# AndreasHeger/gat

Measured on AMD Instinct MI355X. Metric: Monte Carlo samples/sec + bit-exact p-values, 10k sims, hg19-sized workspace, higher is better.
Workload: dtype u32; 1 GPU; config2: 9982 segments x 1 tracks x 9932 intervals, 24 units / 24 contigs, 10000 samples/GPU/step, nucleotide-overlap; steps_in_flight=2

## Files before the change

### gat_amd/csrc/gat_kernels.h

```cpp
#pragma once
#include "gat_device.h"
#include "gat_annotator_steps.h"

namespace gat {


struct SamplerArgs {
  const UnitDev* units;
  const int32_t* order;
  const UnitDev* units_o;
  int32_t n_units;
  int32_t batch;
  int32_t rec_stride;
  const uint2* ws;
  const uint32_t* ws_cdf;
  const uint32_t* rank_len;
  const uint32_t* ws_tree;
  const uint4* ws_rec;
  int4* st2;
  int32_t n_long;
  int32_t n_active;
  uint32_t seed;
  int64_t sample_begin;
  uint2* slab;
// ... 127 lines not shown
            nx[q] = mt[in * kWave];
          }
          if (wv < NT - 1 && k + kGroup == kRngChunk) nx[kGroup - 1] = next_old;
#pragma unroll
          for (int q = 0; q < kGroup; ++q) {
            const uint32_t y = (cur & kMtUpper) | (nx[q] & kMtLower);
            mt[(i0 + k + q) * kWave] = far[q] ^ (y >> 1) ^ ((y & 1u) ? kMtMag : 0u);
            cur = nx[q];
          }
        }
      }
      if (wv < NT - 1) {
        const int tn = NT * (s + 1) + wv + 1;
        next_old = mt[((tn % kPerBlock) * kRngChunk) * kWave];
      }
    } else {
      const int t = NT * (s - 1) + (wv - NT);
      if (t >= 0 && t < nchunks) {
        const int e0 = t * kRngChunk;
        const int cnt = rows - e0 < kRngChunk ? rows - e0 : kRngChunk;
        const uint32_t* __restrict__ src = mt + ((t % kPerBlock) * kRngChunk) * kWave;
        uint32_t* __restrict__ dst = out + (int64_t)e0 * kWave;
        for (int k = 0; k < cnt; k += kGroup) {
          uint32_t w[kGroup];
#pragma unroll
          for (int q = 0; q < kGroup; ++q) w[q] = src[(k + q) * kWave];
#pragma unroll
          for (int q = 0; q < kGroup; ++q) {
#ifndef GAT_RNG_NO_NT
            __builtin_nontemporal_store(mt_temper(w[q]), &dst[(k + q) * kWave]);
#else
            dst[(k + q) * kWave] = mt_temper(w[q]);
#endif
          }
        }
      }
    }
    __syncthreads();
  }
}

constexpr int kPlaceChunk = 8;

template <int KIND, int MODE, int SMALL, bool PIPE>
__device__ __forceinline__ void place_body(const SamplerArgs& A) {
  constexpr bool ALL_SIMPLE = MODE == 1 || MODE == 3;
  constexpr bool TREES = MODE == 2;
  constexpr bool GRID = MODE == 5;
  constexpr int kWsTab = SMALL ? 64 : kPlaceWsLds, kRankTab = MODE == 3 ? 1 : (SMALL == 1 ? 256 : kPlaceRankLds);
  constexpr int WIDE = MODE == 3 ? kPlaceWide : (MODE == 5 ? kPlaceGridTiles : 1);
  __shared__ uint4 l_ws[kWsTab];
  __shared__ uint32_t l_rank_tab[kRankTab];
  __shared__ __attribute__((aligned(8192))) uint2 l_out_all[WIDE][16][kWave];
  extern __shared__ __attribute__((aligned(16))) uint32_t l_rank_wide[];
  uint32_t* const l_rank = MODE == 3 ? l_rank_wide : l_rank_tab;
  const int lane = threadIdx.x & (kWave - 1), wv = __builtin_amdgcn_readfirstlane((int)(threadIdx.x >> 6));
  uint2 (*const l_out)[kWave] = l_out_all[wv];
  const int n_tiles = (A.batch + kWave - 1) / kWave;
  const int a = (int)(blockIdx.y + blockIdx.z * gridDim.y);
  const int sb_own = (int)blockIdx.x * WIDE + wv;
  const int sb = sb_own < n_tiles ? sb_own : n_tiles - 1;
  if (a >= A.n_active) return;
  const UnitDev* __restrict__ Up = A.units_o + a;
  const int nws = Up->n_ws;
  const uint32_t hist_total = Up->hist_total, bucket = Up->bucket, ws_total = Up->ws_total;
  const int cap = Up->slab_cap;
  const uint2* __restrict__ ws = A.ws + Up->ws_off;
  const uint32_t* __restrict__ ws_cdf = A.ws_cdf + Up->ws_off;
  const uint32_t* __restrict__ rank_len = A.rank_len + Up->rank_off;
  const int rows = A.rng_rows[a];
  const int sidx = sb * kWave + lane;
  const bool live = sb_own < n_tiles && sidx < A.batch;
  const int64_t so = GAT_REC(A, sidx, a);

  constexpr bool kind1 = KIND == 1;
  const int target = Up->n_target;
  const bool drawL = hist_total > 2;
  const bool drawP = ws_total > 1;
  if (!drawL || !drawP) {
    if (live) A.st[so] = make_int4(0, Up->ltotal, -1, 0);
    return;
  }
  const uint32_t rangeL = hist_total - 2u, maskL = 0xffffffffu >> __builtin_clz(rangeL);
  const bool drawB = bucket > 1;
  const uint32_t rangeB = bucket - 1u, maskB = drawB ? 0xffffffffu >> __builtin_clz(rangeB) : 0u;
  const uint32_t rangeP = ws_total - 1u, maskP = 0xffffffffu >> __builtin_clz(rangeP);

  {
    const int q = (4 * a) / A.n_active;
    if (q == 0) __builtin_amdgcn_s_setprio(3);
    else if (q == 1) __builtin_amdgcn_s_setprio(2);
    else if (q == 2) __builtin_amdgcn_s_setprio(1);
  }
  const bool ws_lds = nws <= kWsTab;
  const bool rank_lds = MODE == 3 || hist_total < (uint32_t)kRankTab;
  const uint32_t* __restrict__ tree_cdf = A.ws_tree + (Up->tree_cdf_off >= 0 ? Up->tree_cdf_off : 0);
  const WsTreeGeom G = ws_tree_geom(nws);
  if (!ALL_SIMPLE && ws_lds)
    for (int i = lane; i < nws; i += kWave) {
      const uint2 v = ws[i];
      l_ws[i] = make_uint4(ws_cdf[i], v.x, v.y, i > 0 ? ws[i - 1].y : 0x80000000u);
    }
  const uint2 ws0 = ws[0];
  const bool simple_shape = nws == 1 && !drawB && ws0.y - ws0.x > 1u;
  const bool simple_lds = ALL_SIMPLE || (simple_shape && rank_lds);
  if constexpr (MODE == 3) {
    for (int i = (int)threadIdx.x; i <= (int)rangeL; i += WIDE * kWave) l_rank[i] = rank_len[i + 1];
  } else if (simple_lds) {
    for (int i = lane; i <= (int)maskL && i < kRankTab; i += kWave) l_rank[i] = (uint32_t)i <= rangeL ? rank_len[i + 1] : 0u;
  } else if (rank_lds)
    for (int i = lane; i <= (int)hist_total; i += kWave) l_rank[i] = rank_len[i];
  int cshift = 0, cspan = 0;
  uint32_t cmask = 0u;
  const uint16_t* l_g16 = nullptr;
  const uint16_t* l_k16 = nullptr;
  const uint4* __restrict__ wrec = A.ws_rec + Up->ws_off;
  if constexpr (GRID) {
    if (!ws_lds) {
      const uint32_t* __restrict__ cg = A.ws_tree + Up->cgrid_off;
      cshift = (int)cg[0]; cspan = (int)cg[2];
      const int ccells = (int)cg[1], nwords = (int)cg[3];
      cmask = (1u << cshift) - 1u;
      const uint4* __restrict__ src4 = reinterpret_cast<const uint4*>(cg + kGridHeader);
      uint4* dst4 = reinterpret_cast<uint4*>(l_rank_wide);
      for (int i = (int)threadIdx.x; i < (nwords + 3) / 4; i += WIDE * kWave) dst4[i] = src4[i];
      l_g16 = reinterpret_cast<const uint16_t*>(l_rank_wide);
      l_k16 = reinterpret_cast<const uint16_t*>(l_rank_wide + (ccells + 2) / 2);
    }
  }
  __syncthreads();
  bool use_grid = false;
  int gshift = 0, gspan = 0;
  uint8_t* l_grid = reinterpret_cast<uint8_t*>(l_ws + (kWsTab - 9));
  if (!ALL_SIMPLE && ws_lds && !simple_shape && nws > 2 && nws <= kWsTab - 9) {
    const uint32_t top = ws_total - 1u;
    gshift = top >= 128u ? (32 - __builtin_clz(top)) - 7 : 0;
    const int cells = (int)(top >> gshift) + 1;
    for (int c = lane; c <= cells; c += kWave) {
      const uint32_t t = (uint32_t)c << gshift;
      int lo_ = 0, hi_ = nws;
      while (lo_ < hi_) {
        const int mid = lo_ + ((hi_ - lo_) >> 1);
        if ((int32_t)(l_ws[mid].x - t) < 0) lo_ = mid + 1; else hi_ = mid;
      }
      l_grid[c] = (uint8_t)(lo_ < nws ? lo_ : nws - 1);
    }
    __syncthreads();
    uint32_t span = 0;
    for (int c = lane; c < cells; c += kWave) span = max(span, (uint32_t)l_grid[c + 1] - (uint32_t)l_grid[c]);
    gspan = (int)wave_max_u32(span);
    use_grid = true;
  }
  const uint32_t* __restrict__ rp = A.rng_out + A.rng_off[a] + (int64_t)sb * rows * kWave + lane;
  uint2* __restrict__ out = A.slab + (int64_t)(live ? sidx : 0) * A.slab_stride + Up->slab_off;

  int32_t rem = Up->ltotal;
  int nS = 0;
  uint32_t len = 0, cs = 0, ce = 0;
  int32_t sstart = 0;
  int32_t pend = -1;
  uint32_t used = 0;
  int flag = 0;


  bool sL = live, sP = false, sO = false;
  uint32_t omaskS = 0u, orangeS = 0u;
  const int32_t c_ss = (int32_t)ws0.x + 1;
  const uint32_t c_r3 = ws0.y - ws0.x - 2u;
#define GAT_STEP_SIMPLE_B(Y, LR1, JJ)                                                                          \
  {                                                                                                            \
    const uint32_t y_ = (Y);                                                                                   \
        \
    const bool accL = (y_ & maskL) <= rangeL;                                                                  \
    const bool accP = (y_ & maskP) <= rangeP;                                                                  \
              \
    const uint32_t vO = y_ & omaskS;                                                                           \
    const bool accO = vO <= orangeS;                                                                           \
    const bool isL = sL && accL, isP = sP && accP, isO = sO && accO;                                           \
    const uint32_t range3 = c_r3 + len;                                                                        \
    omaskS = isP ? 0xffffffffu >> __builtin_clz(range3 | 1u) : omaskS;                                         \
    orangeS = isP ? range3 : orangeS;                                                                          \
    const bool trig = isL && !kind1 && rem <= (int32_t)(LR1);                         \
    const int32_t q = c_ss - (int32_t)len + (int32_t)vO;                                                       \
    const uint32_t start = (uint32_t)(q > 0 ? q : 0);                                                          \
    const uint32_t end = (uint32_t)(q + (int32_t)len);                                                         \
    const int32_t omin = (int32_t)ws0.y < (int32_t)end ? (int32_t)ws0.y : (int32_t)end;                        \
    const int32_t omax = (int32_t)ws0.x > (int32_t)start ? (int32_t)ws0.x : (int32_t)start;                    \
    const int32_t overlap = omin - omax > 0 ? omin - omax : 0;                                                 \
    const bool full = isO && nS >= cap;                                                                        \
    const bool put = isO && !full;                                                                             \
                                              \
    if (MODE == 3 || put) l_out[nS & 15][lane] = make_uint2(start, end);                                       \
    nS += put ? 1 : 0;                                                                                         \
    rem -= put ? overlap : 0;                                                                                  \
    flag |= full ? kStatusOverflow : 0;                                                                        \
    const bool fin = kind1 && put && nS == target;                                                             \
    len = isL ? (LR1) : len;                                                                                   \
    pend = trig ? (int32_t)len : (fin ? -2 : pend);                                                            \
    used = (trig || put) ? (JJ) + 1u : used;        \
    sL = (sL && !isL) || (put && !fin);                                                                        \
    sP = (sP && !isP) || (isL && !trig);                                                                       \
    sO = (sO && !isO) || isP;                                                                                  \
  }

  const uint32_t lmaxS = rank_len[1u + rangeL];
  const bool cm_ok = A.place_plain_step == 0 && (uint64_t)c_r3 + (uint64_t)lmaxS <= (uint64_t)maskP;
  uint64_t mL = 0, mP = 0, mO = 0;
  uint32_t nS9 = 0, used_lo = 0;
  const uint32_t lane_ring = (uint32_t)(size_t)(__attribute__((address_space(3))) void*)&l_out[0][lane];
#define GAT_STEP_SIMPLE_ASM(YREG, LR1, JJ1)                                                                       \
  {                                                                                                            \
    uint32_t t0_, t1_, t2_, t3_;                                                                               \
    uint64_t sa_, sb_, sc_;                                                                                    \
    asm volatile(                                                                                              \
        "v_and_b32 %7, %16, v" #YREG "\n\t"                                                     \
        "v_and_b32 %8, %26, v" #YREG "\n\t"                                                          \
        "v_cmp_ge_u32_e64 %12, %17, %7\n\t"                                            \
        "v_add_u32 %9, %19, %0\n\t"                                                            \
        "v_cmp_ge_u32 vcc, %18, %8\n\t"                                                              \
        "v_cmp_le_u32_e64 %13, %7, %9\n\t"                                         \
        "s_and_b64 %11, %4, vcc\n\t"                                                                  \
        "v_cmp_le_i32 vcc, %1, %15\n\t"                                  \
        "s_and_b64 %12, %5, %12\n\t"                                                                  \
        "s_and_b64 %13, %6, %13\n\t"                                                                  \
        "s_and_b64 vcc, %11, vcc\n\t"                         \
        "v_cndmask_b32_e64 %0, %0, %15, %11\n\t"                                 \
        "v_cndmask_b32_e64 %3, %3, %25, vcc\n\t"                    \
        "s_xor_b64 %4, %4, %11\n\t"                                                                            \
        "s_andn2_b64 %11, %11, vcc\n\t"                                                   \
        "s_xor_b64 %5, %5, %12\n\t"                                                                            \
        "s_xor_b64 %6, %6, %13\n\t"                                                                            \
        "s_or_b64 %4, %4, %13\n\t"                     \
        "s_or_b64 %5, %5, %11\n\t"                       \
        "s_or_b64 %6, %6, %12\n\t"                                     \
        "s_and_saveexec_b64 %11, %13\n\t"                                 \
        "v_add_u32 %9, %20, %7\n\t"                       \
        "v_and_or_b32 %8, %2, %23, %24\n\t"                                                     \
        "v_sub_u32 %7, %9, %0\n\t"                                                          \
        "v_add_u32 %2, 0x200, %2\n\t"                                                                          \
        "v_min_i32 %10, %22, %9\n\t"                                                     \
        "v_max_i32 %7, 0, %7\n\t"                                                       \
        "v_sub_u32 %1, %1, %10\n\t"                              \
        "v_max_i32 %10, %21, %7\n\t"                                                 \
        "ds_write2_b32 %8, %7, %9 offset1:1\n\t"                                                               \
        "v_mov_b32 %3, %25\n\t"                                                                                \
        "v_add_u32 %1, %1, %10\n\t"                                                                            \
        "s_mov_b64 exec, %11"                                                                                  \
        : "+v"(len), "+v"(rem), "+v"(nS9), "+v"(used_lo), "+s"(mL), "+s"(mP), "+s"(mO),                        \
          "=&v"(t0_), "=&v"(t1_), "=&v"(t2_), "=&v"(t3_), "=&s"(sa_), "=&s"(sb_), "=&s"(sc_)                   \
        : "n"(0), "v"(LR1), "s"(maskP), "s"(rangeP), "s"(rangeL), "s"(c_r3), "s"(c_ss), "s"(ws0.x), "s"(ws0.y), \
          "s"(0x1e00u), "v"(lane_ring), "n"(JJ1), "s"(maskL)                                                   \
        : "vcc", "scc", "memory");                                                                             \
  }

  int nF = 0;
  auto flush = [&]() __attribute__((always_inline)) {
    if (nS - nF >= 8 && nF + 8 <= cap) {
      uint4* __restrict__ dst = reinterpret_cast<uint4*>(out + nF);
      const int w0 = nF & 15;
#pragma unroll
      for (int w = 0; w < 4; ++w) {
        const uint2 e0 = l_out[w0 + 2 * w][lane], e1 = l_out[w0 + 2 * w + 1][lane];
#ifdef GAT_EXP_NO_STORES
        if (e0.x == 0xfffffff1u && e1.y == 0xfffffff2u)
#endif
        dst[w] = make_uint4(e0.x, e0.y, e1.x, e1.y);
      }
      nF += 8;
    }
  };
  bool sB = false;
  bool alive_c = true;
  uint32_t omask = 0u, orange = 0u;
#define GAT_STEP_TABLE_B(Y, LR, PCS, PCE, PPE, JJ)                                                             \
  {                                                                                                            \
    const uint32_t y_ = (Y);                                                                                   \
    const uint32_t vB = y_ & maskB, vO = y_ & omask;                                                           \
    const bool isL = sL && (y_ & maskL) <= rangeL, isB = sB && vB <= rangeB;                                   \
    const bool isP = sP && (y_ & maskP) <= rangeP, isO = sO && vO <= orange;                                   \
    len = isL ? (LR) * bucket : (isB ? len + vB : len);                                          \
    const bool have_len = drawB ? isB : isL;                                                                   \
    const bool trig = have_len && !kind1 && rem <= (int32_t)len;                      \
    cs = isP ? (PCS) : cs;                                                                                     \
    ce = isP ? (PCE) : ce;                                                                                     \
    int32_t sstartP = (int32_t)(PCS) - (int32_t)len + 1;                                         \
    sstartP = (int32_t)(PPE) > sstartP ? (int32_t)(PPE) : sstartP;                                             \
    const uint32_t range3 = (PCE) - 1u - (uint32_t)sstartP;                                                    \
    const bool placeP = isP && range3 == 0;                             \
    const bool place = isO || placeP;                                                                          \
    const int32_t q = isO ? sstart + (int32_t)vO : sstartP;                                                    \
    const uint32_t start = (uint32_t)(q > 0 ? q : 0);                                  \
    const uint32_t end = (uint32_t)(q + (int32_t)len);                                                         \
    const int32_t omin = (int32_t)ce < (int32_t)end ? (int32_t)ce : (int32_t)end;                              \
    const int32_t omax = (int32_t)cs > (int32_t)start ? (int32_t)cs : (int32_t)start;                          \
    const int32_t overlap = omin - omax > 0 ? omin - omax : 0;                                                 \
    const bool full = place && nS >= cap;                                                                      \
    const bool put = place && !full;                                                                           \
    if (put) l_out[nS & 15][lane] = make_uint2(start, end);                                                    \
    nS += put ? 1 : 0;                                                                                         \
    rem -= put ? overlap : 0;                                                                                  \
    flag |= full ? kStatusOverflow : 0;                                                                        \
    const bool fin = kind1 && put && nS == target;                                                             \
    pend = trig ? (int32_t)len : (fin ? -2 : pend);                                                            \
    used = (trig || put) ? (JJ) + 1u : used;                                                                   \
    sstart = isP ? sstartP : sstart;                                                                           \
    omask = isP ? 0xffffffffu >> __builtin_clz(range3 | 1u) : omask;                                           \
    orange = isP ? range3 : orange;                                                                            \
    sL = (sL && !isL) || (put && !fin);                                                                        \
    sB = (sB && !isB) || (isL && drawB);                                                                       \
    sP = (sP && !isP) || (have_len && !trig);                                                                  \
    sO = (sO && !isO) || (isP && !placeP);                                                                     \
  }

  uint32_t ya[kPlaceChunk], yb[kPlaceChunk], lr[kPlaceChunk] = {0, 0, 0, 0, 0, 0, 0, 0};
  uint32_t pcs[kPlaceChunk] = {0, 0, 0, 0, 0, 0, 0, 0}, pce[kPlaceChunk] = {0, 0, 0, 0, 0, 0, 0, 0},
           ppe[kPlaceChunk] = {0, 0, 0, 0, 0, 0, 0, 0};
#define GAT_STEP_TABLE_ASM(YREG, LR1, PCS, PCE, PPE, JJ1)                                                         \
  {                                                                                                            \
    uint32_t t0_, t1_, t2_, t3_;                                                                               \
    uint64_t sa_, sb_, sc_;                                                                                    \
    asm volatile(                                                                                              \
        "v_and_b32 %12, %24, v" #YREG "\n\t"                                                         \
        "v_and_b32 %13, %27, v" #YREG "\n\t"                                                         \
        "v_and_b32 %14, %8, v" #YREG "\n\t"                                    \
        "v_cmp_ge_u32_e64 %17, %25, %12\n\t"                                                         \
        "v_cmp_ge_u32 vcc, %26, %13\n\t"                                                             \
        "v_cmp_le_u32_e64 %18, %14, %9\n\t"                                         \
        "s_and_b64 %16, %4, vcc\n\t"                                                                  \
        "v_cmp_le_i32 vcc, %1, %20\n\t"                                  \
        "s_and_b64 %17, %5, %17\n\t"                                                                  \
        "s_and_b64 %18, %6, %18\n\t"                                                                  \
        "s_and_b64 vcc, %16, vcc\n\t"                                                      \
        "v_cndmask_b32_e64 %0, %0, %20, %16\n\t"                                                      \
        "v_cndmask_b32_e64 %3, %3, %30, vcc\n\t"                                                  \
        "s_xor_b64 %4, %4, %16\n\t"                                                                            \
        "s_andn2_b64 %16, %16, vcc\n\t"                                                   \
        "s_xor_b64 %5, %5, %17\n\t"                                                                            \
        "s_xor_b64 %6, %6, %18\n\t"                                                                            \
        "s_or_b64 %5, %5, %16\n\t"                               \
        "s_and_saveexec_b64 %16, %17\n\t"                       \
        "v_sub_u32 %12, %21, %0\n\t"                                                  \
        "v_mov_b32 %10, %21\n\t"                                                                       \
        "v_add_u32 %12, 1, %12\n\t"                                                                            \
        "v_mov_b32 %11, %22\n\t"                                                                       \
        "v_max_i32 %7, %23, %12\n\t"                                                       \
        "v_mov_b32 %14, 0\n\t"                              \
        "v_sub_u32 %12, %22, %7\n\t"                                                                           \
        "v_add_u32 %9, -1, %12\n\t"                    \
        "v_or_b32 %12, 1, %9\n\t"                                                                              \
        "v_ffbh_u32 %12, %12\n\t"                                                                              \
        "v_cmp_eq_u32 vcc, 0, %9\n\t"                                             \
        "v_lshrrev_b32_e64 %8, %12, -1\n\t"                                                      \
        "s_mov_b64 exec, %16\n\t"                                                                              \
        "s_andn2_b64 %17, %17, vcc\n\t"                                                 \
        "s_or_b64 %18, %18, vcc\n\t"                                                 \
        "s_or_b64 %6, %6, %17\n\t"                                           \
        "s_or_b64 %4, %4, %18\n\t"                                               \
        "s_and_saveexec_b64 %16, %18\n\t"                                                                      \
        "v_add_u32 %12, %7, %14\n\t"                                          \
        "v_and_or_b32 %13, %2, %28, %29\n\t"                                                    \
        "v_add_u32 %15, %12, %0\n\t"                                                        \
        "v_max_i32 %12, 0, %12\n\t"                                                     \
        "v_add_u32 %2, 0x200, %2\n\t"                                                                          \
        "v_min_i32 %14, %11, %15\n\t"                                                        \
        "v_sub_u32 %1, %1, %14\n\t"                                                  \
        "v_max_i32 %14, %10, %12\n\t"                                                      \
        "ds_write2_b32 %13, %12, %15 offset1:1\n\t"                                                            \
        "v_mov_b32 %3, %30\n\t"                                                                                \
        "v_add_u32 %1, %1, %14\n\t"                                                                            \
        "s_mov_b64 exec, %16"                                                                                  \
        : "+v"(len), "+v"(rem), "+v"(nS9), "+v"(used_lo), "+s"(mL), "+s"(mP), "+s"(mO),                        \
          "+v"(sstart), "+v"(omask), "+v"(orange), "+v"(cs), "+v"(ce),                                         \
          "=&v"(t0_), "=&v"(t1_), "=&v"(t2_), "=&v"(t3_), "=&s"(sa_), "=&s"(sb_), "=&s"(sc_)                   \
        : "n"(0), "v"(LR1), "v"(PCS), "v"(PCE), "v"(PPE), "s"(maskP), "s"(rangeP), "s"(rangeL), "s"(maskL),    \
          "s"(0x1e00u), "v"(lane_ring), "n"(JJ1)                                                               \
        : "vcc", "scc", "memory");                                                                             \
  }
#define GAT_PRE_RANK_L(Y)                                                                                      \
  _Pragma("unroll") for (int c = 0; c < kPlaceChunk; ++c) {                                                    \
    const uint32_t v = (Y)[c] & maskL; lr[c] = l_rank[v <= rangeL ? 1u + v : 0u]; }
#define GAT_PRE_RANK_G(Y)                                                                                      \
  _Pragma("unroll") for (int c = 0; c < kPlaceChunk; ++c) {                                                    \
    const uint32_t v = (Y)[c] & maskL; lr[c] = rank_len[v <= rangeL ? 1u + v : 0u]; }
#define GAT_PRE_WS(Y)                                                                                          \
  {                                                                                                            \
    uint32_t pv[kPlaceChunk]; int lo[kPlaceChunk];                                                             \
    _Pragma("unroll") for (int c = 0; c < kPlaceChunk; ++c) {                                                  \
      const uint32_t v = (Y)[c] & maskP; pv[c] = v <= rangeP ? v : rangeP; lo[c] = 0; }                        \
    if (use_grid) {                                                                                            \
      _Pragma("unroll") for (int c = 0; c < kPlaceChunk; ++c) lo[c] = (int)l_grid[pv[c] >> gshift];             \
    }                                                                                                          \
    for (int n = use_grid ? gspan : nws; n > 1;) {              \
      const int half = n >> 1;                                                                                 \
      _Pragma("unroll") for (int c = 0; c < kPlaceChunk; ++c) {                                                \
        const int pr = lo[c] + half - 1;                 \
        lo[c] = (int32_t)(l_ws[pr < nws ? pr : nws - 1].x - pv[c]) < 0 ? lo[c] + half : lo[c];                 \
      }                                                                                                        \
      n -= half;                                                                                               \
    }                                                                                                          \
    _Pragma("unroll") for (int c = 0; c < kPlaceChunk; ++c) {                                                  \
      uint4 w4 = l_ws[lo[c]];                                                                                  \
      if ((int32_t)(w4.x - pv[c]) < 0) w4 = l_ws[lo[c] + 1];                                                   \
      pcs[c] = w4.y; pce[c] = w4.z; ppe[c] = w4.w; }                                                           \
  }
#define GAT_PRE_WS2(Y)                                                                                         \
  {                                                                                                            \
    uint32_t pv[kPlaceChunk]; int lo[kPlaceChunk];                                                             \
    _Pragma("unroll") for (int c = 0; c < kPlaceChunk; ++c) {                                                  \
      const uint32_t v = (Y)[c] & maskP; pv[c] = v <= rangeP ? v : rangeP; }                                   \
    {                                                        \
      const uint32_t pa[4] = {pv[0], pv[1], pv[2], pv[3]}, pb[4] = {pv[4], pv[5], pv[6], pv[7]};               \
      int la[4], lb[4];                                                                                        \
      ws_tree_count<true, 4>(tree_cdf, G, pa, la);                                                             \
      ws_tree_count<true, 4>(tree_cdf, G, pb, lb);                                                             \
      _Pragma("unroll") for (int c = 0; c < 4; ++c) { lo[c] = la[c]; lo[4 + c] = lb[c]; }                      \
    }                                                                                                          \
    _Pragma("unroll") for (int c = 0; c < kPlaceChunk; ++c) {                                                  \
      const uint2 w2 = ws[lo[c]];                                                                              \
      pcs[c] = w2.x; pce[c] = w2.y; ppe[c] = lo[c] > 0 ? ws[lo[c] - 1].y : 0x80000000u; }                      \
  }
#ifdef GAT_EXP_NOGATHER
#define GAT_EXP_REC(I) ((I) & 0)
#else
// ... 212 lines not shown
    int jbase = 0;                                                                                           \
    uint32_t pcsB[kPlaceChunk], pceB[kPlaceChunk], ppeB[kPlaceChunk];                                        \
    asm volatile("; GAT_PINNED_BEGIN BASE=192" ::: "memory");                                                \
    GAT_PIN_LOAD(192, 193, 194, 195, 196, 197, 198, 199, 0)                                                  \
    GAT_PIN_LOAD(200, 201, 202, 203, 204, 205, 206, 207, kPlaceChunk)                                        \
    GAT_PIN_LOAD(208, 209, 210, 211, 212, 213, 214, 215, 2 * kPlaceChunk)                                    \
    GAT_PIN_LOAD(216, 217, 218, 219, 220, 221, 222, 223, 3 * kPlaceChunk)                                    \
    GAT_PIN_TAKE2(ya, 192, 193, 194, 195, 196, 197, 198, 199)                                                \
    alive_c = sL;                                                                                            \
    GAT_PRE_WS3X(ya, pcs, pce, ppe)                                                                          \
    for (int j = 0; j < rows; j += 4 * kPlaceChunk) {                                                        \
      if ((mL | mP | mO) == 0) break;                                                                        \
      GAT_FOLD_USED(jbase)                                                                                   \
      jbase = j;                                                                                             \
      GAT_DEEP_SUB(0, ya, pcs, pce, ppe, yb, pcsB, pceB, ppeB, 200, 201, 202, 203, 204, 205, 206, 207,        \
                   192, 193, 194, 195, 196, 197, 198, 199, j + 4 * kPlaceChunk)                               \
      if (j + 1 * kPlaceChunk >= rows || (mL | mP | mO) == 0) break;                                         \
      GAT_DEEP_SUB(1, yb, pcsB, pceB, ppeB, ya, pcs, pce, ppe, 208, 209, 210, 211, 212, 213, 214, 215,        \
                   200, 201, 202, 203, 204, 205, 206, 207, j + 5 * kPlaceChunk)                               \
      if (j + 2 * kPlaceChunk >= rows || (mL | mP | mO) == 0) break;                                         \
      GAT_DEEP_SUB(2, ya, pcs, pce, ppe, yb, pcsB, pceB, ppeB, 216, 217, 218, 219, 220, 221, 222, 223,        \
                   208, 209, 210, 211, 212, 213, 214, 215, j + 6 * kPlaceChunk)                               \
      if (j + 3 * kPlaceChunk >= rows || (mL | mP | mO) == 0) break;                                         \
      GAT_DEEP_SUB(3, yb, pcsB, pceB, ppeB, ya, pcs, pce, ppe, 192, 193, 194, 195, 196, 197, 198, 199,        \
                   216, 217, 218, 219, 220, 221, 222, 223, j + 7 * kPlaceChunk)                               \
    }                                                                                                        \
    asm volatile("s_waitcnt vmcnt(0)\n\t; GAT_PINNED_END" ::: "memory");                                     \
    GAT_FOLD_USED(jbase)                                                                                     \
    nS = (int)(nS9 >> 9);                                                                                    \
    sL = (mL >> lane) & 1; sP = (mP >> lane) & 1; sO = (mO >> lane) & 1;                                     \
  }
#define GAT_PLACE_LOOP(PRE, ONE, ALIVE)                                                                        \
  {                                                                                                            \
    const uint32_t* __restrict__ rq = rp;                                                                      \
    _Pragma("unroll") for (int c = 0; c < kPlaceChunk; ++c) ya[c] = rq[c * kWave];                             \
    for (int j = 0; j < rows; j += 2 * kPlaceChunk) {                                                          \
      if (__ballot(ALIVE) == 0) break;                                                                         \
      GAT_PSTAMP(4)                                                                                            \
      const bool more_b = j + kPlaceChunk < rows;                                                              \
      if (more_b) {                                                                                            \
        _Pragma("unroll") for (int c = 0; c < kPlaceChunk; ++c) yb[c] = rq[(kPlaceChunk + c) * kWave];         \
      }                                                                                                        \
      GAT_PSTAMP(0)                                                                                            \
      if constexpr (GRID) alive_c = (ALIVE);                                                                   \
      PRE(ya)                                                                                                  \
      GAT_PSTAMP(1)                                                                                            \
      _Pragma("unroll") for (int c = 0; c < kPlaceChunk; ++c) ONE(ya, c, (uint32_t)(j + c))                    \
      GAT_PSTAMP(2)                                                                                            \
      GAT_PSTAMP(3)                                                                                            \
      GAT_PROWS                                                                                                \
      if (!more_b || __ballot(ALIVE) == 0) break;                                                              \
      if (j + 2 * kPlaceChunk < rows) {                                                                        \
        _Pragma("unroll") for (int c = 0; c < kPlaceChunk; ++c) ya[c] = rq[(2 * kPlaceChunk + c) * kWave];     \
      }                                                                                                        \
      rq += 2 * kPlaceChunk * kWave;                                                                           \
      GAT_PSTAMP(0)                                                                                            \
      if constexpr (GRID) alive_c = (ALIVE);                                                                   \
      PRE(yb)                                                                                                  \
      GAT_PSTAMP(1)                                                                                            \
      _Pragma("unroll") for (int c = 0; c < kPlaceChunk; ++c) ONE(yb, c, (uint32_t)(j + kPlaceChunk + c))      \
      GAT_PSTAMP(2)                                                                                            \
      flush();                                                                                                 \
      GAT_PSTAMP(3)                                                                                            \
      GAT_PROWS                                                                                                \
    }                                                                                                          \
  }
  bool plain_step = true;
  if constexpr (MODE == 3) {
    static_assert(PIPE, "k_place_wide runs the hand-pipelined loop");
    if (!kind1 && cm_ok) { plain_step = false; GAT_PLACE_LOOP_PIPE_ASM(GAT_PRE_SIMPLE_W, GAT_ONE_SIMPLE_ASM) }
    else GAT_PLACE_LOOP_PIPE(GAT_PRE_SIMPLE_W, GAT_ONE_SIMPLE_B, GAT_ALIVE_B)
  } else if (simple_lds) {
    if constexpr (PIPE) {
      if (!kind1 && cm_ok) { plain_step = false; GAT_PLACE_LOOP_PIPE_ASM(GAT_PRE_SIMPLE_L, GAT_ONE_SIMPLE_ASM) }
      else GAT_PLACE_LOOP_PIPE(GAT_PRE_SIMPLE_L, GAT_ONE_SIMPLE_B, GAT_ALIVE_B)
    } else GAT_PLACE_LOOP(GAT_PRE_SIMPLE_L, GAT_ONE_SIMPLE_B, GAT_ALIVE_B)
  } else if constexpr (!ALL_SIMPLE) {
    if (simple_shape) GAT_PLACE_LOOP(GAT_PRE_SIMPLE_G, GAT_ONE_SIMPLE_B, GAT_ALIVE_B)
    else {
      if (ws_lds) {
        if (rank_lds) {
          if (!kind1 && !drawB && A.place_plain_step == 0) { plain_step = false; GAT_PLACE_LOOP_PIPE_ASM(GAT_PRE_TABLE_LL, GAT_ONE_TABLE_ASM) }
          else GAT_PLACE_LOOP(GAT_PRE_TABLE_LL, GAT_ONE_TABLE, GAT_ALIVE_TB)
        } else GAT_PLACE_LOOP(GAT_PRE_TABLE_GL, GAT_ONE_TABLE, GAT_ALIVE_TB)
      } else if constexpr (TREES) {
        if (rank_lds) GAT_PLACE_LOOP(GAT_PRE_TABLE_LG, GAT_ONE_TABLE, GAT_ALIVE_TB) else GAT_PLACE_LOOP(GAT_PRE_TABLE_GG, GAT_ONE_TABLE, GAT_ALIVE_TB)
      } else if constexpr (GRID) {
        if (rank_lds) {
          if (!kind1 && !drawB && A.place_plain_step == 0) {
            plain_step = false;
            GAT_PLACE_LOOP_DEEP_ASM
          } else GAT_PLACE_LOOP(GAT_PRE_TABLE_L3, GAT_ONE_TABLE, GAT_ALIVE_TB)
        } else GAT_PLACE_LOOP(GAT_PRE_TABLE_G3, GAT_ONE_TABLE, GAT_ALIVE_TB)
      }
    }
  }
#undef GAT_PROWS
#ifdef GAT_DIAG
  if (lane == 0 && A.diag_place != nullptr && sb_own < n_tiles) {
    for (int k = 0; k < 5; ++k) atomicAdd(&A.diag_place[(int64_t)a * 8 + k], pdg[k]);
    atomicAdd(&A.diag_place[(int64_t)a * 8 + 5], pdg_rows);
    atomicAdd(&A.diag_place[(int64_t)a * 8 + 6], 1ull);
    if (A.diag_tiles != nullptr) {
      unsigned long long tile_t1;
      asm volatile("s_memrealtime %0\n\ts_waitcnt lgkmcnt(0)" : "=s"(tile_t1) :: "memory");
      A.diag_tiles[((int64_t)a * n_tiles + sb_own) * 2] = tile_t0;
      A.diag_tiles[((int64_t)a * n_tiles + sb_own) * 2 + 1] = tile_t1;
    }
  }
#endif
#undef GAT_PLACE_LOOP
#undef GAT_PLACE_LOOP_PIPE
#undef GAT_PLACE_CHUNK
#undef GAT_PIN_TAKE
#undef GAT_PIN_LOAD
#undef GAT_ONE_TABLE
#undef GAT_ONE_SIMPLE_B
#undef GAT_ALIVE_B
#undef GAT_STEP_SIMPLE_B
#undef GAT_STEP_SIMPLE_ASM
#undef GAT_STEP_TABLE_ASM
#undef GAT_ONE_SIMPLE_ASM
#undef GAT_ONE_TABLE_ASM
#undef GAT_PLACE_LOOP_PIPE_ASM
#undef GAT_PLACE_CHUNK_ASM
#undef GAT_FOLD_USED
#undef GAT_PRE_TABLE_GG
#undef GAT_PRE_TABLE_L3
#undef GAT_PRE_TABLE_G3
#undef GAT_PRE_WS3
#undef GAT_PRE_WS3X
#undef GAT_PLACE_LOOP_DEEP_ASM
#undef GAT_DEEP_SUB
#undef GAT_ONE_TABLE_ASM2
#undef GAT_PIN_TAKE2
#undef GAT_PRE_TABLE_LG
#undef GAT_PRE_TABLE_GL
#undef GAT_PRE_TABLE_LL
#undef GAT_PRE_SIMPLE_G
#undef GAT_PRE_SIMPLE_W
#undef GAT_PRE_SIMPLE_L
#undef GAT_PRE_WS2
#undef GAT_PRE_WS
#undef GAT_PRE_RANK_G
#undef GAT_PRE_RANK_L
#undef GAT_STEP_TABLE_B
#undef GAT_ALIVE_TB
  if (live) {
    const bool halted = !(sL || sB || sP || sO);
    if (!plain_step) {
      if (!kind1 && halted) pend = (int32_t)len;
      if (nS > cap) { flag |= kStatusOverflow; nS = nF; }
    }
    for (int i = nF; i < nS; ++i) out[i] = l_out[i & 15][lane];
    A.st[so] = make_int4(nS, rem, flag != 0 ? -1 : (halted ? (pend != -1 ? pend : -1) : (kind1 ? -1 : -3)), (int)used);
    if (flag) atomicOr(A.flags, flag);
  }
}

template <int KIND, int MODE, int SMALL = 0>
__global__ __launch_bounds__(64) __attribute__((amdgpu_waves_per_eu(MODE == 0 && SMALL == 1 ? 4 : 1))) void k_place(SamplerArgs A) {
  place_body<KIND, MODE, SMALL, false>(A);
}

template <int KIND, int MODE, int SMALL = 0>
__global__ __launch_bounds__(64) __attribute__((amdgpu_num_vgpr(96), amdgpu_waves_per_eu(MODE == 0 && SMALL == 1 ? 4 : 1))) void k_place_pipe(SamplerArgs A) {
  place_body<KIND, MODE, SMALL, true>(A);
}

template <int KIND>
__global__ __launch_bounds__(kPlaceWide * 64) void k_place_wide(SamplerArgs A) {
  place_body<KIND, 3, 0, true>(A);
}

__global__ __launch_bounds__(kPlaceGridTiles * 64) void k_place_grid(SamplerArgs A) {
  place_body<0, 5, 0, true>(A);
}

#ifndef GAT_SCAN_WAVES
#define GAT_SCAN_WAVES 8
#endif
constexpr int kScanStreams = 16, kScanWaves = GAT_SCAN_WAVES, kScanPer = kScanStreams / kScanWaves, kScanPitch = kWave + 1;
constexpr int kScanRankTab = kPlaceRankLds;
constexpr int kFnIdentity = 0x03020100;

__device__ __forceinline__ int scan_fn_compose(int a, int b) {
  return (int)__builtin_amdgcn_perm(0u, (uint32_t)a, (uint32_t)b);
}

struct ScanStream {
  uint32_t state8;
  uint32_t len;
  int32_t rem;
  int32_t nS;
  uint32_t used;
  int32_t pend;
  int32_t flag;
  bool done;
};

struct ScanUnit {
  uint32_t maskL, rangeL, maskP, rangeP, c_r3;
  int32_t c_ss, ws_start, ws_end, cap;
};

__device__ __forceinline__ void place_scan_chunk(ScanStream& T, const ScanUnit& U, uint32_t y, uint32_t lr, int nrows, uint32_t row0,
                                                 uint2* __restrict__ out, int lane, bool pessimist) {
  const bool in = lane < nrows;
  const uint32_t vO = y & U.maskP;
  const bool aL = in && (y & U.maskL) <= U.rangeL, aP = in && vO <= U.rangeP;
  bool aO = in && !pessimist && vO <= U.c_r3 + 1u;
  const uint64_t lt = lanemask_lt(lane), le = lt | (1ull << lane);
  const int fLP = 0x03000000 | (aL ? 1 : 0) | ((aP ? 2 : 1) << 8);
  int Fi;
  uint32_t len;
  bool isL, isO;
  uint64_t bL;
  for (;;) {
    const int f = fLP | ((aO ? 0 : 2) << 16);
    Fi = wave_incl_scan_dpp(f, kFnIdentity, [](int a, int b) { return scan_fn_compose(a, b); });
    const int Fe = __builtin_amdgcn_update_dpp(kFnIdentity, Fi, 0x138, 0xf, 0xf, false);
    const uint32_t st = __builtin_amdgcn_ubfe((uint32_t)Fe, T.state8, 8);
    isL = aL && st == 0u;
    bL = __ballot(isL);
    const uint64_t mL = bL & le;
    const int src = mL ? 63 - __builtin_clzll(mL) : lane;
    const uint32_t got = (uint32_t)__builtin_amdgcn_ds_bpermute(src << 2, (int)lr);
    len = mL ? got : T.len;
    const bool exact = in && vO <= U.c_r3 + len;
    isO = aO && st == 2u;
    if (!__any(st == 2u && exact != aO)) break;
    aO = st == 2u ? exact : aO;
  }
  const int32_t q = U.c_ss - (int32_t)len + (int32_t)vO;
  const uint32_t start = (uint32_t)(q > 0 ? q : 0), end = (uint32_t)(q + (int32_t)len);
  const int32_t omin = U.ws_end < (int32_t)end ? U.ws_end : (int32_t)end, omax = U.ws_start > (int32_t)start ? U.ws_start : (int32_t)start;
  const uint32_t ov = isO ? (uint32_t)(omin - omax > 0 ? omin - omax : 0) : 0u;
  const uint32_t incl = wave_incl_sum_u32(ov, lane);
  const int32_t rem_before = T.rem - (int32_t)(incl - ov);
  const bool trig = isL && rem_before <= (int32_t)lr;
  const uint64_t bT = __ballot(trig);
  const int jt = bT ? __builtin_ctzll(bT) : kWave - 1;
  const uint64_t keep = bT ? ((1ull << jt) - 1ull) : ~0ull;
  const uint64_t bO = __ballot(isO) & keep;
  const int idx = T.nS + (int)__builtin_amdgcn_mbcnt_hi((uint32_t)(bO >> 32), __builtin_amdgcn_mbcnt_lo((uint32_t)bO, 0u));
  const int nput = __popcll(bO);
  const bool over = T.nS + nput > U.cap;
  if (!over && ((bO >> lane) & 1ull)) out[idx] = make_uint2(start, end);
  const int32_t rem_t = __builtin_amdgcn_readlane(rem_before, jt), lr_t = __builtin_amdgcn_readlane((int)lr, jt);
  const int32_t tot = __builtin_amdgcn_readlane((int)incl, kWave - 1);
  const uint32_t len_end = bL ? (uint32_t)__builtin_amdgcn_readlane((int)lr, 63 - __builtin_clzll(bL)) : T.len;
  const uint32_t st_end = 8u * __builtin_amdgcn_ubfe((uint32_t)__builtin_amdgcn_readlane(Fi, kWave - 1), T.state8, 8);
  const uint32_t used_put = bO ? row0 + (uint32_t)(63 - __builtin_clzll(bO)) + 1u : T.used;
  T.flag |= over ? kStatusOverflow : 0;
  T.done = over || bT != 0;
  if (!over) {
    T.nS += nput;
    T.used = bT ? row0 + (uint32_t)jt + 1u : used_put;
    T.pend = bT ? lr_t : T.pend;
    T.rem = bT ? rem_t : T.rem - tot;
    T.len = len_end;
    T.state8 = st_end;
  }
}

__global__ __launch_bounds__(kScanWaves * 64) void k_place_scan(SamplerArgs A, int n_sb, int pessimist) {
  __shared__ uint32_t l_rows[2][kScanStreams * kScanPitch];
  __shared__ uint32_t l_rank[kScanRankTab];
  __shared__ int32_t l_live[2][kScanWaves];
  const int lane = threadIdx.x & (kWave - 1), wv = __builtin_amdgcn_readfirstlane((int)(threadIdx.x >> 6));
  const int64_t n_tiles = (int64_t)n_sb * A.n_active;
  const int64_t b = blockIdx.x, slot = b >> 3;
  const int64_t tile = (slot >> 2) * 8 + (b & 7);
  const int quarter = (int)(slot & 3);
  if (tile >= n_tiles) return;
  const int a = (int)(tile / n_sb), sb = (int)(tile % n_sb);
  const UnitDev* __restrict__ Up = A.units_o + a;
  const uint32_t hist_total = Up->hist_total, ws_total = Up->ws_total;
  const int rows = A.rng_rows[a];
  const uint2 ws0 = A.ws[Up->ws_off];
  const uint32_t* __restrict__ rank_len = A.rank_len + Up->rank_off;
  const int col0 = quarter * kScanStreams;
  ScanUnit U;
  ScanStream T[kScanPer];
  uint2* outp[kScanPer];
  int64_t so[kScanPer];
  bool live[kScanPer];
  const bool degenerate = !(hist_total > 2 && ws_total > 1);
#pragma unroll
  for (int q = 0; q < kScanPer; ++q) {
    const int sidx = sb * kWave + col0 + wv * kScanPer + q;
    live[q] = sidx < A.batch;
    so[q] = GAT_REC(A, live[q] ? sidx : 0, a);
    outp[q] = A.slab + (int64_t)(live[q] ? sidx : 0) * A.slab_stride + Up->slab_off;
    T[q].state8 = 0u; T[q].len = 0u; T[q].rem = Up->ltotal; T[q].nS = 0; T[q].used = 0u; T[q].pend = -1; T[q].flag = 0;
    T[q].done = !live[q];
  }
  if (degenerate) {
#pragma unroll
    for (int q = 0; q < kScanPer; ++q)
      if (live[q] && lane == 0) A.st[so[q]] = make_int4(0, Up->ltotal, -1, 0);
    return;
  }
  U.rangeL = hist_total - 2u; U.maskL = 0xffffffffu >> __builtin_clz(U.rangeL);
  U.rangeP = ws_total - 1u; U.maskP = 0xffffffffu >> __builtin_clz(U.rangeP);
  U.c_ss = (int32_t)ws0.x + 1; U.c_r3 = ws0.y - ws0.x - 2u;
// ... 2062 lines not shown
```

Before: 4.602 million samples/s.

## Cooperatively flush ready lanes' staged segments via wave-wide compaction

The per-lane flush, where each ready lane wrote 8 segments as 4 uint4 stores to its own slab row, is replaced by a wave-cooperative flush. Ready lanes are compacted with ballot, mbcnt and ds_permute, then four lanes share each owner's 64-byte chunk, so each store instruction writes contiguous 64B runs instead of 64 scattered 16B pieces. This should give better store coalescing, at the cost of extra cross-lane permutes and a loop over ready lanes on every flush call. The address calculation now assumes slab rows for sample sb*kWave+lane, which replaces the live/sidx indexing.

Result: no change. 4.634 million samples/s, median of 6 (+0.7%).

```diff
diff --git a/gat_amd/csrc/gat_kernels.h b/gat_amd/csrc/gat_kernels.h
--- a/gat_amd/csrc/gat_kernels.h
+++ b/gat_amd/csrc/gat_kernels.h
@@ -303,7 +303,12 @@
     use_grid = true;
   }
   const uint32_t* __restrict__ rp = A.rng_out + A.rng_off[a] + (int64_t)sb * rows * kWave + lane;
+#ifdef GAT_FLUSH_PER_LANE
   uint2* __restrict__ out = A.slab + (int64_t)(live ? sidx : 0) * A.slab_stride + Up->slab_off;
+#else
+  uint2* const out_tile = A.slab + (int64_t)sb * kWave * A.slab_stride + Up->slab_off;
+  auto slab_of = [&](int l) __attribute__((always_inline)) { return out_tile + (int64_t)l * A.slab_stride; };
+#endif
 
   int32_t rem = Up->ltotal;
   int nS = 0;
@@ -405,6 +410,31 @@
   }
 
   int nF = 0;
+#ifndef GAT_FLUSH_PER_LANE
+  auto flush = [&]() __attribute__((always_inline)) {
+    const bool ready = nS - nF >= 8 && nF + 8 <= cap;
+    const uint64_t rb = __ballot(ready);
+    if (rb == 0) return;
+    const int R = __builtin_popcountll(rb);
+    const int rk = (int)__builtin_amdgcn_mbcnt_hi((uint32_t)(rb >> 32), __builtin_amdgcn_mbcnt_lo((uint32_t)rb, 0u));
+    const int sent = __builtin_amdgcn_ds_permute((ready ? rk : R + lane - rk) << 2, (int)(((uint32_t)nF << 3) | (uint32_t)lane));
+    const int q = lane & 3;
+    for (int it = 0; it * 16 < R; ++it) {
+      const int r = it * 16 + (lane >> 2);
+      const uint32_t w = (uint32_t)__builtin_amdgcn_ds_bpermute(r << 2, sent);
+      if (r < R) {
+        const int owner = (int)(w & 63u), nFo = (int)((w >> 6) << 3);
+        const int s0 = (nFo & 15) + 2 * q;
+        const uint2 e0 = l_out[s0][owner], e1 = l_out[s0 + 1][owner];
+#ifdef GAT_EXP_NO_STORES
+        if (e0.x == 0xfffffff1u && e1.y == 0xfffffff2u)
+#endif
+        reinterpret_cast<uint4*>(slab_of(owner) + nFo)[q] = make_uint4(e0.x, e0.y, e1.x, e1.y);
+      }
+    }
+    nF += ready ? 8 : 0;
+  };
+#else
   auto flush = [&]() __attribute__((always_inline)) {
     if (nS - nF >= 8 && nF + 8 <= cap) {
       uint4* __restrict__ dst = reinterpret_cast<uint4*>(out + nF);
@@ -420,6 +450,7 @@
       nF += 8;
     }
   };
+#endif
   bool sB = false;
   bool alive_c = true;
   uint32_t omask = 0u, orange = 0u;
@@ -938,6 +969,9 @@
       if (!kind1 && halted) pend = (int32_t)len;
       if (nS > cap) { flag |= kStatusOverflow; nS = nF; }
     }
+#ifndef GAT_FLUSH_PER_LANE
+    uint2* __restrict__ out = slab_of(lane);
+#endif
     for (int i = nF; i < nS; ++i) out[i] = l_out[i & 15][lane];
     A.st[so] = make_int4(nS, rem, flag != 0 ? -1 : (halted ? (pend != -1 ? pend : -1) : (kind1 ? -1 : -3)), (int)used);
     if (flag) atomicOr(A.flags, flag);
```
